# Bostanabad-Research-Group/GP-Plus

Measured on AMD Instinct MI355X. Metric: MLL evals/sec (fwd+grad), NxN exact GP, N=20k d=8, higher is better.
Workload: dtype f64; 1 GPU; C2: synthetic Borehole (Sobol seed 0, unique rows, z-scored) N=20000 d=8 fp64, GP_Plus Rough_RBF exact GP at theta1, one replica per GPU (restart-parallel); N=20000, d=8, streams_per_gpu=1

## Files before the change

gp-plus_amd/csrc/gpp_gemm.hip:

```cpp
#include "../../include/gpp.h"
#include "gpp_internal.h"

#include <algorithm>
#include <atomic>
#include <cstdlib>

typedef double v2d __attribute__((ext_vector_type(2)));
typedef double v4d __attribute__((ext_vector_type(4)));

namespace {

constexpr int BK16 = 16;
constexpr int ldt_mc(int T, int BK = 16) { return BK == 16 ? T + 16 : T + 4; }
constexpr int LDK = BK16 + 2;

__device__ __forceinline__ bool keep_elem(int mask, int k, int row) {
  return (mask == 0) | ((mask == 1) & (k <= row)) | ((mask == 2) & (k >= row));
}

template <int T>
__device__ __forceinline__ unsigned load_kc(const double* __restrict__ P, int64_t ld, int R, int r0, int kb, int kend,
                                            int mask, int tid, v2d (&reg)[T / 32]) {
  unsigned keep = 0;
  const double* ptr[T / 32];
#pragma unroll
  for (int i = 0; i < T / 32; ++i) {
    const int v = tid + 256 * i;
    const int gr = r0 + (v >> 3);
    const int gk = kb + ((v & 7) << 1);
    const bool v0 = (gr < R) & (gk < kend);
    const bool k0 = v0 & keep_elem(mask, gk, gr);
    const bool k1 = v0 & (gk + 1 < kend) & keep_elem(mask, gk + 1, gr);
    keep |= (k0 ? 1u : 0u) << (2 * i);
    keep |= (k1 ? 1u : 0u) << (2 * i + 1);
    ptr[i] = v0 ? P + (int64_t)gr * ld + gk : P;
  }
#pragma unroll
  for (int i = 0; i < T / 32; ++i) reg[i] = *reinterpret_cast<const v2d*>(ptr[i]);
  return keep;
}
template <int T, bool SEL>
__device__ __forceinline__ void store_kc(double* __restrict__ s, int tid, const v2d (&reg)[T / 32], unsigned keep) {
#pragma unroll
  for (int i = 0; i < T / 32; ++i) {
    const int v = tid + 256 * i;
    v2d t = reg[i];
    if (SEL) {
      t.x = ((keep >> (2 * i)) & 1u) ? t.x : 0.0;
      t.y = ((keep >> (2 * i + 1)) & 1u) ? t.y : 0.0;
    }
    *reinterpret_cast<v2d*>(s + (v >> 3) * LDK + ((v & 7) << 1)) = t;
  }
}

template <int T, int BK, int NTH = 256>
__device__ __forceinline__ unsigned load_mc(const double* __restrict__ P, int64_t ld, int R, int r0, int kb, int kend,
                                            int mask, int tid, v2d (&reg)[BK * T / (2 * NTH)], const double* __restrict__ dummy) {
  constexpr int NV = BK * T / (2 * NTH);
  unsigned keep = 0;
  const double* ptr[NV];
#pragma unroll
  for (int i = 0; i < NV; ++i) {
    const int v = tid + NTH * i;
    const int gk = kb + v / (T / 2);
    const int gr = r0 + ((v % (T / 2)) << 1);
    const bool v0 = (gk < kend) & (gr < R);
    const bool k0 = v0 & keep_elem(mask, gk, gr);
    const bool k1 = v0 & (gr + 1 < R) & keep_elem(mask, gk, gr + 1);
    keep |= (k0 ? 1u : 0u) << (2 * i);
    keep |= (k1 ? 1u : 0u) << (2 * i + 1);
    ptr[i] = v0 ? P + (int64_t)gk * ld + gr : dummy;
  }
#pragma unroll
  for (int i = 0; i < NV; ++i) reg[i] = *reinterpret_cast<const v2d*>(ptr[i]);
  return keep;
}
template <int T, int BK, bool SEL, int NTH = 256>
__device__ __forceinline__ void store_mc(double* __restrict__ s, int tid, const v2d (&reg)[BK * T / (2 * NTH)], unsigned keep) {
#pragma unroll
  for (int i = 0; i < BK * T / (2 * NTH); ++i) {
    const int v = tid + NTH * i;
    v2d t = reg[i];
    if (SEL) {
      t.x = ((keep >> (2 * i)) & 1u) ? t.x : 0.0;
      t.y = ((keep >> (2 * i + 1)) & 1u) ? t.y : 0.0;
    }
    *reinterpret_cast<v2d*>(s + (v / (T / 2)) * ldt_mc(T, BK) + ((v % (T / 2)) << 1)) = t;
  }
}

template <int T, int BK>
__device__ __forceinline__ bool chunk_is_interior(int r0, int R, int kb, int kend, int mask) {
  if (r0 + T > R || kb + BK > kend) return false;
  if (mask == 1) return kb + BK - 1 <= r0;
  if (mask == 2) return kb >= r0 + T - 1;
  return true;
}
template <int T, int BK>
__device__ __forceinline__ bool chunk_in_range(int r0, int R, int kb, int kend) {
  return r0 + T <= R && kb + BK <= kend;
}
template <int T, int BK, int NTH = 256>
__device__ __forceinline__ unsigned mask_bits_mc(int r0, int kb, int mask, int tid) {
  unsigned keep = 0;
#pragma unroll
  for (int i = 0; i < BK * T / (2 * NTH); ++i) {
    const int v = tid + NTH * i;
    const int gk = kb + v / (T / 2);
    const int gr = r0 + ((v % (T / 2)) << 1);
    keep |= (keep_elem(mask, gk, gr) ? 1u : 0u) << (2 * i);
    keep |= (keep_elem(mask, gk, gr + 1) ? 1u : 0u) << (2 * i + 1);
  }
  return keep;
}
template <int T, bool KC, int BK, int NTH = 256>
__device__ __forceinline__ void thread_offsets(int64_t ld, int tid, unsigned (&off)[BK * T / (2 * NTH)]) {
#pragma unroll
  for (int i = 0; i < BK * T / (2 * NTH); ++i) {
    const int v = tid + NTH * i;
    if (KC) off[i] = (unsigned)(((int64_t)(v >> 3) * ld + ((v & 7) << 1)) * 8);
    else off[i] = (unsigned)(((int64_t)(v / (T / 2)) * ld + ((v % (T / 2)) << 1)) * 8);
  }
}
template <int NV>
__device__ __forceinline__ void load_fast(const double* __restrict__ ubase, const unsigned (&off)[NV], v2d (&reg)[NV]) {
#pragma unroll
  for (int i = 0; i < NV; ++i)
    reg[i] = *reinterpret_cast<const v2d*>(reinterpret_cast<const char*>(ubase) + off[i]);
}

struct GemmNoHook {
  __device__ __forceinline__ void operator()() const {}
};
struct GemmStoreC {};
template <int VAR, int WTM, int WTN, int TAG, int BK, int NBUF, int WR, class P, class H = GemmNoHook, class E = GemmStoreC>
__device__ __forceinline__ void gemm_tile(const P& p, const int tm, const int tn, const double* __restrict__ A,
                                          const double* __restrict__ B, double* __restrict__ C, double* C2,
                                          double* __restrict__ smem, H before_epilogue = H(), const E& epi = E()) {
  static_assert(BK == 16 || VAR == 2, "wide K chunks are implemented for row-contiguous (TN) operands only");
  static_assert(BK % 16 == 0 && (NBUF == 1 || NBUF == 2), "bad staging parameters");
  static_assert(WR == 2 || (WR == 4 && VAR == 2 && BK == 16 && NBUF == 2 && WTM == 64 && WTN == 64), "the tall tile is TN only");
  constexpr int NTH = 128 * WR;
  constexpr bool A_KC = (VAR != 2);
  constexpr bool B_KC = (VAR == 0);
  constexpr int TM = WR * WTM, TN = 2 * WTN;
  constexpr int LDA = ldt_mc(TM, BK), LDB = ldt_mc(TN, BK);
  constexpr int TX = TM > TN ? TM : TN;
  constexpr int OPSZ = (BK * ldt_mc(TX, BK) > TX * LDK) ? BK * ldt_mc(TX, BK) : TX * LDK;
  constexpr int OPA = (WR == 2) ? OPSZ : BK * LDA, OPB = (WR == 2) ? OPSZ : BK * LDB;
  constexpr int NVA = BK * TM / (2 * NTH), NVB = BK * TN / (2 * NTH);
  constexpr int RB = WTM / 4, CB = WTN / 16;

  const int tid = threadIdx.x;
  const int wave = tid >> 6, lane = tid & 63;
  const int wm = (wave >> 1) * WTM, wn = (wave & 1) * WTN;
  const int li = lane & 15, lk = lane >> 4;
  const int row0 = tm * TM, col0 = tn * TN;
  const double* __restrict__ Bd = B;
  double* __restrict__ Cd = C;
  if (p.compact_bc) {
    const int b = tn / p.own_bt, q = (b + p.own_off) / p.own_mod;
    const int64_t bias = (int64_t)(q - b) * p.own_bt * TN;
    B += bias;
    C += bias;
  }

  int klo = 0;
  if (p.klo_mode == 1) klo = row0;
  else if (p.klo_mode == 2) klo = col0;
  else if (p.klo_mode == 3) klo = row0 > col0 ? row0 : col0;
  int khi = p.K;
  if (p.khi_mode == 1) khi = min(p.K, row0 + TM);
  else if (p.khi_mode == 2) khi = min(p.K, col0 + TN);
  const int nch = khi > klo ? (khi - klo + BK - 1) / BK : 0;

  static_assert(RB % 4 == 0, "wave tile rows must be a multiple of 16");
  v4d acc4[RB / 4][CB];
#pragma unroll
  for (int a = 0; a < RB / 4; ++a)
#pragma unroll
    for (int b = 0; b < CB; ++b) acc4[a][b] = (v4d){0.0, 0.0, 0.0, 0.0};

  v2d ra[NVA], rb[NVB];
  unsigned ka = 0, kb_ = 0;
  unsigned offa[NVA], offb[NVB];
  thread_offsets<TM, A_KC, BK, NTH>(p.lda, tid, offa);
  thread_offsets<TN, B_KC, BK, NTH>(p.ldb, tid, offb);
  const double* __restrict__ ubaseA = A_KC ? A + (int64_t)row0 * p.lda : A + row0;
  const double* __restrict__ ubaseB = B_KC ? B + (int64_t)col0 * p.ldb : B + col0;
  const int64_t stepA = A_KC ? 1 : p.lda, stepB = B_KC ? 1 : p.ldb;

  const int Mld = (VAR == 2 && p.pad_ok) ? ((p.M + TM - 1) / TM) * TM : p.M;
  const int Nld = (VAR == 2 && p.pad_ok) ? ((p.N + TN - 1) / TN) * TN : p.N;
  int pa = 0, pb = 0;
  auto stage_load = [&](int kb) {
    pa = pb = 0;
    if constexpr (VAR == 2) {
      if (chunk_in_range<TM, BK>(row0, Mld, kb, khi)) pa = chunk_is_interior<TM, BK>(row0, Mld, kb, khi, p.a_mask) ? 1 : 2;
      if (chunk_in_range<TN, BK>(col0, Nld, kb, khi)) pb = chunk_is_interior<TN, BK>(col0, Nld, kb, khi, p.b_mask) ? 1 : 2;
    }
    if (pa) {
      load_fast<NVA>(ubaseA + (int64_t)kb * stepA, offa, ra);
      if (pa == 2) ka = mask_bits_mc<TM, BK, NTH>(row0, kb, p.a_mask, tid);
    } else {
      if constexpr (A_KC) ka = load_kc<TM>(A, p.lda, p.M, row0, kb, khi, p.a_mask, tid, ra);
      else ka = load_mc<TM, BK, NTH>(A, p.lda, p.M, row0, kb, khi, p.a_mask, tid, ra, A);
    }
    if (pb) {
      load_fast<NVB>(ubaseB + (int64_t)kb * stepB, offb, rb);
      if (pb == 2) kb_ = mask_bits_mc<TN, BK, NTH>(col0, kb, p.b_mask, tid);
    } else {
      if constexpr (B_KC) kb_ = load_kc<TN>(B, p.ldb, p.N, col0, kb, khi, p.b_mask, tid, rb);
      else kb_ = load_mc<TN, BK, NTH>(B, p.ldb, p.N, col0, kb, khi, p.b_mask, tid, rb, Bd);
    }
  };
  auto stage_store = [&](double* da, double* db) {
    if (pa == 1) {
      if constexpr (A_KC) store_kc<TM, false>(da, tid, ra, 0); else store_mc<TM, BK, false, NTH>(da, tid, ra, 0);
    } else {
      if constexpr (A_KC) store_kc<TM, true>(da, tid, ra, ka); else store_mc<TM, BK, true, NTH>(da, tid, ra, ka);
    }
    if (pb == 1) {
      if constexpr (B_KC) store_kc<TN, false>(db, tid, rb, 0); else store_mc<TN, BK, false, NTH>(db, tid, rb, 0);
    } else {
      if constexpr (B_KC) store_kc<TN, true>(db, tid, rb, kb_); else store_mc<TN, BK, true, NTH>(db, tid, rb, kb_);
    }
  };

  auto kpos = [&](int c) { return p.k_reverse ? klo + (nch - 1 - c) * BK : klo + c * BK; };
  if (nch > 0) {
    stage_load(kpos(0));
    stage_store(smem, smem + OPA);
  }
  __syncthreads();

  auto compute = [&](int cur) {
    const double* sa = smem + cur * (OPA + OPB) + (A_KC ? (wm + li) * LDK + lk : wm + li + lk * LDA);
    const double* sb = smem + cur * (OPA + OPB) + OPA + (B_KC ? (wn + li) * LDK + lk : wn + li + lk * LDB);
#pragma unroll
    for (int kk = 0; kk < BK / 4; ++kk) {
      double bf[CB], af[RB / 4];
#pragma unroll
      for (int b = 0; b < CB; ++b) bf[b] = B_KC ? sb[16 * b * LDK + kk * 4] : sb[kk * 4 * LDB + 16 * b];
#pragma unroll
      for (int a = 0; a < RB / 4; ++a) af[a] = A_KC ? sa[16 * a * LDK + kk * 4] : sa[kk * 4 * LDA + 16 * a];
#pragma unroll
      for (int a = 0; a < RB / 4; ++a)
#pragma unroll
        for (int b = 0; b < CB; ++b)
          acc4[a][b] = __builtin_amdgcn_mfma_f64_16x16x4f64(af[a], bf[b], acc4[a][b], 0, 0, 0);
    }
  };

  int ca = 0, cb = 0;
  constexpr bool SPLIT = (VAR == 2 && RB == 16 && CB == 4 && BK == 16);
  if constexpr (SPLIT) {
    if (row0 + TM <= Mld && col0 + TN <= Nld && nch > 1) {
      int k_lo = klo, k_hi = khi;
      if (p.a_mask == 1) k_hi = min(k_hi, row0 + 1);
      if (p.a_mask == 2) k_lo = max(k_lo, row0 + TM - 1);
      if (p.b_mask == 1) k_hi = min(k_hi, col0 + 1);
      if (p.b_mask == 2) k_lo = max(k_lo, col0 + TN - 1);
      int j_lo = (k_lo - klo + BK - 1) / BK, j_hi = (k_hi - klo) / BK;
      j_lo = max(j_lo, 0);
      j_hi = min(j_hi, nch);
      if (j_hi > j_lo) {
        const int ci_lo = p.k_reverse ? nch - j_hi : j_lo, ci_hi = p.k_reverse ? nch - j_lo : j_hi;
        ca = max(ci_lo - 1, 0);
        cb = min(ci_hi - 1, nch - 1);
        if (cb < ca) ca = cb = 0;
      }
    }
  }
  auto general_iter = [&](int c) {
    const int cur = (NBUF == 2) ? (c & 1) : 0;
    const bool more = (c + 1 < nch);
    if (more) stage_load(kpos(c + 1));
    compute(cur);
    if (NBUF == 1) __syncthreads();
    if (more) {
      const int nxt = (NBUF == 2) ? (cur ^ 1) : 0;
      stage_store(smem + nxt * (OPA + OPB), smem + nxt * (OPA + OPB) + OPA);
    }
    __syncthreads();
  };
  int c = 0;
  for (; c < ca; ++c) general_iter(c);
  if constexpr (SPLIT) {
    for (; c < cb; ++c) {
      const int cur = (NBUF == 2) ? (c & 1) : 0, nxt = (NBUF == 2) ? (cur ^ 1) : 0;
      const int kb = kpos(c + 1);
      load_fast<NVA>(ubaseA + (int64_t)kb * stepA, offa, ra);
      load_fast<NVB>(ubaseB + (int64_t)kb * stepB, offb, rb);
      if constexpr (TAG != 0) __builtin_amdgcn_s_setprio(1);
      compute(cur);
      if constexpr (TAG != 0) __builtin_amdgcn_s_setprio(0);
      if (NBUF == 1) __syncthreads();
      store_mc<TM, BK, false, NTH>(smem + nxt * (OPA + OPB), tid, ra, 0);
      store_mc<TN, BK, false, NTH>(smem + nxt * (OPA + OPB) + OPA, tid, rb, 0);
      __syncthreads();
    }
  }
  for (; c < nch; ++c) general_iter(c);
  before_epilogue();
  if constexpr (!__is_same(E, GemmStoreC)) {
    static_assert((VAR == 2 || VAR == 0) && WTM == 64 && WTN == 64 && WR == 2, "accumulator epilogues are written for the big tile");
    epi(acc4, row0, col0, p.M, smem);
    return;
  }

  const double alpha = p.alpha, beta = p.beta;
  constexpr int GA = RB < 4 ? RB : 4;
#pragma unroll
  for (int a0 = 0; a0 < RB; a0 += GA) {
    double cold[GA][CB];
    if (beta != 0.0) {
#pragma unroll
      for (int a = 0; a < GA; ++a) {
        const int m = row0 + wm + 4 * (a0 + a) + lk;
#pragma unroll
        for (int b = 0; b < CB; ++b) {
          const int n = col0 + wn + 16 * b + li;
          const bool ok = (m < p.M) && (n < p.N) && (p.c_lower == 0 || (p.c_lower == 1 ? n <= m : n >= m));
          const double* src = ok ? C + (int64_t)m * p.ldc + n : Cd;
          cold[a][b] = *src;
        }
      }
    }
#pragma unroll
    for (int a = 0; a < GA; ++a) {
      const int m = row0 + wm + 4 * (a0 + a) + lk;
#pragma unroll
      for (int b = 0; b < CB; ++b) {
        const int n = col0 + wn + 16 * b + li;
        const bool ok = (m < p.M) && (n < p.N) && (p.c_lower == 0 || (p.c_lower == 1 ? n <= m : n >= m));
        double v = alpha * acc4[(a0 + a) >> 2][b][(a0 + a) & 3];
        if (beta != 0.0) v = fma(beta, cold[a][b], v);
        if (ok) {
          C[(int64_t)m * p.ldc + n] = v;
          if (C2)
            C2[(int64_t)n * p.ldc2 + m] = v;
        }
      }
    }
  }
}

template <int VAR, int WTM, int WTN, int TAG = 0, int BK = 16, int NBUF = 2, int WR = 2>
__global__ __launch_bounds__(128 * WR, ((VAR == 2 && !(BK > 16 && WTM >= 64)) || WTM < 64) ? 2 : 1) void gpp_gemm_f64(GemmArgs p) {
  constexpr int TM = WR * WTM, TN = 2 * WTN;
  extern __shared__ __attribute__((aligned(16))) double smem[];
  int tm, tn;
  if (p.swz) {
    const int b = blockIdx.x, xcd = b & 7, i = b >> 3;
    const int S = (i >> 6) * 8 + xcd, w = i & 63;
    const int super_n = (p.tiles_n + 7) >> 3;
    const int sm = S / super_n, sn = S - sm * super_n;
    tm = sm * 8 + (w >> 3);
    tn = sn * 8 + (w & 7);
    if (tm >= p.tiles_m || tn >= p.tiles_n) return;
    if ((p.c_lower == 1 && tn > tm) || (p.c_lower == 2 && tn < tm)) return;
  } else {
    const int t = (p.batch_fast ? (int)(blockIdx.x / (unsigned)p.nbatch) : (int)blockIdx.x) + (int)p.tile_base;
    if (p.c_lower == 1 && p.row_mod >= 1) {
      const float a = 0.5f * (float)p.row_mod, b = (float)p.row_off + 1.f - a;
      int i = (int)((-b + sqrtf(b * b + 4.f * a * (float)t)) / (2.f * a));
      auto S = [&](int q) { return q * (p.row_off + 1) + p.row_mod * (q * (q - 1) / 2); };
      while (S(i + 1) <= t) ++i;
      while (S(i) > t) --i;
      tm = p.row_off + p.row_mod * i;
      tn = t - S(i);
    } else if (p.c_lower == 1 && TM == 2 * TN) {
      tm = (int)((sqrtf(4.f * (float)t + 1.f) - 1.f) * 0.5f);
      while ((tm + 1) * (tm + 2) <= t) ++tm;
      while (tm * (tm + 1) > t) --tm;
      tn = t - tm * (tm + 1);
      if (tn >= p.tiles_n) return;
    } else if (p.c_lower) {
      tm = (int)((sqrtf(8.f * (float)t + 1.f) - 1.f) * 0.5f);
      while ((tm + 1) * (tm + 2) / 2 <= t) ++tm;
      while (tm * (tm + 1) / 2 > t) --tm;
      tn = t - tm * (tm + 1) / 2;
      if (p.c_lower == 1 && p.own_mod > 1 && (tn / p.own_bt + p.own_off) % p.own_mod != 0) return;
      if (p.c_lower == 2) {
        const int q = tm;
        tm = tn;
        tn = q;
        if (p.own_mod > 1 && (tm / p.own_bt + p.own_off) % p.own_mod != 0) return;
        if ((tn + 1) * TN <= p.skip_lead) return;
        if (p.row_limit > 0 && tm * TM >= p.row_limit) return;
      }
    } else if (p.col_major) {
      tn = t / p.tiles_m;
      tm = t - tn * p.tiles_m;
    } else {
      tm = t / p.tiles_n;
      tn = t - tm * p.tiles_n;
      if (p.row_reverse) tm = p.tiles_m - 1 - tm;
    }
  }
  const int64_t bi = p.batch_fast ? (int64_t)(blockIdx.x % (unsigned)p.nbatch) : (int64_t)blockIdx.y;
  gemm_tile<VAR, WTM, WTN, TAG, BK, NBUF, WR>(p, tm, tn, p.A + bi * p.sA + (int64_t)blockIdx.z * p.zA, p.B + bi * p.sB + (int64_t)blockIdx.z * p.zB,
                                             p.C + bi * p.sC + (int64_t)blockIdx.z * p.zC,
                                             p.C2 ? p.C2 + bi * p.sC2 + (int64_t)blockIdx.z * p.zC2 : nullptr, smem);

}

__device__ __forceinline__ double wave_sum(double v) {
#pragma unroll
  for (int o = 32; o > 0; o >>= 1) v += __shfl_xor(v, o);
  return v;
}
template <int DT>
struct GradEpilogue {
  GradEpiArgs e;
  int tile;
  static constexpr int T = 128;
  static constexpr int FIXED = 2 * DT * T + 2 * T + DT + 4 * (DT + 1);
  static constexpr int SLAB = (FIXED + 1) & ~1;
  static_assert((SLAB + 16 * 256) * sizeof(double) <= 2 * 2 * BK16 * ldt_mc(T) * sizeof(double), "the epilogue lives in the main loop's LDS");
  __device__ __forceinline__ void operator()(const v4d (&acc4)[4][4], int row0, int col0, int N, double* __restrict__ smem) const {
    const int tid = threadIdx.x, wave = tid >> 6, lane = tid & 63;
    const int wm = (wave >> 1) * 64, wn = (wave & 1) * 64, li = lane & 15, lk = lane >> 4;
    const int D = e.D;
    double* __restrict__ sa = smem;
    double* __restrict__ sb = sa + DT * T;
    double* __restrict__ sal_a = sb + DT * T;
    double* __restrict__ sal_b = sal_a + T;
    double* __restrict__ sw = sal_b + T;
    double* __restrict__ red = sw + DT;
    double* __restrict__ slab = smem + SLAB;
    for (int x = tid; x < DT * T; x += 256) {
      const int d = x / T, r = x - d * T;
      sa[x] = (d < D && row0 + r < N) ? e.U[(int64_t)(row0 + r) * D + d] : 0.0;
      sb[x] = (d < D && col0 + r < N) ? e.U[(int64_t)(col0 + r) * D + d] : 0.0;
    }
    if (tid < T) {
      sal_a[tid] = (row0 + tid < N) ? e.alpha[row0 + tid] : 0.0;
      sal_b[tid] = (col0 + tid < N) ? e.alpha[col0 + tid] : 0.0;
    }
    if (tid < DT) sw[tid] = (tid < D) ? e.w[tid] : 0.0;
    __syncthreads();

    const double sf2 = *e.sf2;
    const GppExpConsts ec = gpp_exp_consts();
    const bool diag_tile = (row0 == col0);
    double my_sf2 = 0.0, my_w[DT];
#pragma unroll
    for (int d = 0; d < DT; ++d) my_w[d] = 0.0;
#pragma unroll
    for (int a4 = 0; a4 < 4; ++a4) {
#pragma unroll
      for (int v = 0; v < 4; ++v)
#pragma unroll
        for (int b = 0; b < 4; ++b) slab[(v * 4 + b) * 256 + tid] = acc4[a4][b][v];
#pragma unroll 1
      for (int h = 0; h < 2; ++h) {
        const int ra = wm + 16 * a4 + 8 * h + lk;
        const int cb = wn + li;
        double r2[2][4];
#pragma unroll
        for (int a = 0; a < 2; ++a)
#pragma unroll
          for (int b = 0; b < 4; ++b) r2[a][b] = 0.0;
#pragma unroll 2
        for (int d = 0; d < DT; ++d) {
          const double ua[2] = {sa[d * T + ra], sa[d * T + ra + 4]};
          const double wd = sw[d];
#pragma unroll
          for (int b = 0; b < 4; ++b) {
            const double ub = sb[d * T + cb + 16 * b];
#pragma unroll
            for (int a = 0; a < 2; ++a) {
              const double df = ua[a] - ub;
              r2[a][b] = fma(wd * df, df, r2[a][b]);
            }
          }
        }
        __asm__ volatile("" ::: "memory");
        double g2[2][4];
#pragma unroll
        for (int a = 0; a < 2; ++a) {
          const int i = row0 + ra + 4 * a;
          const double al_i = sal_a[ra + 4 * a];
#pragma unroll
          for (int b = 0; b < 4; ++b) {
            const int j = col0 + cb + 16 * b;
            const bool ok = (i < N) & (j <= i);
            const double kv = gpp_exp_nonpos(-r2[a][b], ec);
            const double kin = slab[((2 * h + a) * 4 + b) * 256 + tid];
            double Wij = 0.5 * (al_i * sal_b[cb + 16 * b] - kin);
            Wij = ok ? Wij : 0.0;
            const double mult = (i == j) ? 1.0 : 2.0;
            my_sf2 = fma(mult * Wij, kv, my_sf2);
            g2[a][b] = mult * Wij * sf2 * kv;
            if (diag_tile && ok && i == j) e.wdiag[i] = Wij;
          }
        }
#pragma unroll
        for (int d = 0; d < DT; ++d) {
          const double ua[2] = {sa[d * T + ra], sa[d * T + ra + 4]};
          double s = 0.0;
#pragma unroll
          for (int b = 0; b < 4; ++b) {
            const double ub = sb[d * T + cb + 16 * b];
#pragma unroll
            for (int a = 0; a < 2; ++a) {
              const double df = ua[a] - ub;
              s = fma(-g2[a][b] * df, df, s);
            }
          }
          my_w[d] += s;
          __builtin_amdgcn_sched_barrier(0);
        }
      }
    }
#pragma unroll
    for (int q = 0; q <= DT; ++q) {
      const double v = wave_sum(q < DT ? my_w[q < DT ? q : 0] : my_sf2);
      if (lane == 0) red[wave * (DT + 1) + q] = v;
    }
    __syncthreads();
    if (tid <= D) {
      const int q = (tid == D) ? DT : tid;
      e.rec[(int64_t)tile * (D + 1) + tid] = ((red[q] + red[(DT + 1) + q]) + red[2 * (DT + 1) + q]) + red[3 * (DT + 1) + q];
    }
  }
};

template <int DT>
__global__ __launch_bounds__(256, 2) void gpp_lauum_grad_f64(GemmArgs p, GradEpiArgs e) {
  extern __shared__ __attribute__((aligned(16))) double smem[];
  const int t = (int)blockIdx.x;
  int tm = (int)((sqrtf(8.f * (float)t + 1.f) - 1.f) * 0.5f);
  while ((tm + 1) * (tm + 2) / 2 <= t) ++tm;
  while (tm * (tm + 1) / 2 > t) --tm;
  const int tn = t - tm * (tm + 1) / 2;
  gemm_tile<2, 64, 64, 2, 16, 2, 2>(p, tm, tn, p.A, p.B, nullptr, nullptr, smem, GemmNoHook(), GradEpilogue<DT>{e, t});
}

template <bool MAT>
struct PostCrossEpilogue {
  PostCrossArgs e;
  int tile, Mr;
  static constexpr int T = 128, DC = 16;
  static constexpr int SLAB = 2 * DC * T + T + 2 * T;
  static_assert((SLAB & 1) == 0 && (SLAB + 16 * 256) * sizeof(double) <= 2 * 2 * BK16 * ldt_mc(T) * sizeof(double) &&
                    (SLAB + 16 * 256) * sizeof(double) <= 2 * 2 * T * LDK * sizeof(double),
                "the epilogue lives in the main loop's LDS");
  __device__ __forceinline__ void operator()(const v4d (&acc4)[4][4], int row0, int col0, int Mc, double* __restrict__ smem) const {
    const int tid = threadIdx.x, wave = tid >> 6, lane = tid & 63;
    const int wm = (wave >> 1) * 64, wn = (wave & 1) * 64, li = lane & 15, lk = lane >> 4;
    const int D = e.dk & 255, kind = (e.dk >> 8) & 255;
    const int dsp = (!MAT || kind == 0) ? D : (e.dk >> 16);
    double* __restrict__ sa = smem;
    double* __restrict__ sb = sa + DC * T;
    double* __restrict__ som = sb + DC * T;
    double* __restrict__ rs = som + T;
    double* __restrict__ slab = smem + SLAB;
    const double* __restrict__ Uc = e.Uc;
    const double* __restrict__ Ur = e.Ur;
    const double* __restrict__ wp = e.w;
    double* __restrict__ rec = e.rec + (int64_t)tile * T;
    Uc += (int64_t)row0 * (e.dk & 255);
    Ur += (int64_t)col0 * (e.dk & 255);
    int rlim = Mc - row0, clim = Mr - col0;
    asm volatile("" : "+v"(Uc), "+v"(Ur), "+v"(wp), "+v"(rec), "+v"(rlim), "+v"(clim));
    auto stage = [&](int d0) {
      for (int x = tid; x < DC * T; x += 256) {
        const int dd = x / T, r = x - dd * T, d = d0 + dd;
        const bool okd = d < D;
        const double sw = okd ? sqrt(wp[okd ? d : 0]) : 0.0;
        sa[x] = (okd && r < rlim) ? Uc[r * D + d] * sw : 0.0;
        sb[x] = (okd && r < clim) ? Ur[r * D + d] * sw : 0.0;
      }
    };
    if (tid < T) som[tid] = (tid < clim) ? (e.omega ? e.omega[col0 + tid] : 1.0) : 0.0;
    const bool one = (D <= DC);
    if (one) stage(0);
    __syncthreads();

    const double sf2 = *e.sf2;
    const GppExpConsts ec = gpp_exp_consts();
#pragma unroll
    for (int a4 = 0; a4 < 4; ++a4) {
#pragma unroll
      for (int v = 0; v < 4; ++v)
#pragma unroll
        for (int b = 0; b < 4; ++b) slab[(v * 4 + b) * 256 + tid] = acc4[a4][b][v];
#pragma unroll 1
      for (int h = 0; h < 2; ++h) {
        const int ra = wm + 16 * a4 + 8 * h + lk;
        const int cb = wn + li;
        double r2[2][4], r2m[MAT ? 2 : 1][MAT ? 4 : 1];
#pragma unroll
        for (int a = 0; a < 2; ++a)
#pragma unroll
          for (int b = 0; b < 4; ++b) {
            r2[a][b] = 0.0;
            if (MAT) r2m[MAT ? a : 0][MAT ? b : 0] = 0.0;
          }
#pragma unroll 1
        for (int d0 = 0; d0 < D; d0 += DC) {
// ... 733 lines not shown
```

Baseline: 7.961 evals/s.

## Hand-schedule interior GEMM k-loop to interleave global loads, LDS ops and MFMAs

Adds a dedicated pipelined main loop for interior tiles of the TN double-buffered big-tile GEMM. It uses scalar-uniform base pointers with per-thread offsets, register-fragment prefetch of the next k-step, and explicit sched_group_barrier ordering that spreads global loads, LDS reads and LDS writes between MFMAs. The goal is to hide memory and LDS latency behind matrix math and reduce address arithmetic. It adds compiler-sensitive scheduling code and asm register pinning that may raise register pressure or serialize poorly if the schedule mismatches the generated instructions.

```diff
diff --git a/gp-plus_amd/csrc/gpp_gemm.hip b/gp-plus_amd/csrc/gpp_gemm.hip
--- a/gp-plus_amd/csrc/gpp_gemm.hip
+++ b/gp-plus_amd/csrc/gpp_gemm.hip
@@ -7,9 +7,14 @@
 
 typedef double v2d __attribute__((ext_vector_type(2)));
 typedef double v4d __attribute__((ext_vector_type(4)));
+typedef const char __attribute__((address_space(1))) gchar;
+typedef const v2d __attribute__((address_space(1))) gv2d;
 
 namespace {
 
+#ifndef GPP_CLEAN_SETPRIO
+#define GPP_CLEAN_SETPRIO 1
+#endif
 constexpr int BK16 = 16;
 constexpr int ldt_mc(int T, int BK = 16) { return BK == 16 ? T + 16 : T + 4; }
 constexpr int LDK = BK16 + 2;
@@ -150,6 +155,8 @@
   constexpr int OPA = (WR == 2) ? OPSZ : BK * LDA, OPB = (WR == 2) ? OPSZ : BK * LDB;
   constexpr int NVA = BK * TM / (2 * NTH), NVB = BK * TN / (2 * NTH);
   constexpr int RB = WTM / 4, CB = WTN / 16;
+  constexpr bool SPLIT = (VAR == 2 && RB == 16 && CB == 4 && BK == 16 && NBUF == 2 && WR == 2);
+  constexpr bool PIPE = SPLIT && __is_same(H, GemmNoHook);
 
   const int tid = threadIdx.x;
   const int wave = tid >> 6, lane = tid & 63;
@@ -199,6 +206,12 @@
       if (chunk_in_range<TM, BK>(row0, Mld, kb, khi)) pa = chunk_is_interior<TM, BK>(row0, Mld, kb, khi, p.a_mask) ? 1 : 2;
       if (chunk_in_range<TN, BK>(col0, Nld, kb, khi)) pb = chunk_is_interior<TN, BK>(col0, Nld, kb, khi, p.b_mask) ? 1 : 2;
     }
+    if constexpr (PIPE) {
+#pragma unroll
+      for (int i = 0; i < NVA; ++i) asm("" : "+v"(offa[i]));
+#pragma unroll
+      for (int i = 0; i < NVB; ++i) asm("" : "+v"(offb[i]));
+    }
     if (pa) {
       load_fast<NVA>(ubaseA + (int64_t)kb * stepA, offa, ra);
       if (pa == 2) ka = mask_bits_mc<TM, BK, NTH>(row0, kb, p.a_mask, tid);
@@ -253,7 +266,6 @@
   };
 
   int ca = 0, cb = 0;
-  constexpr bool SPLIT = (VAR == 2 && RB == 16 && CB == 4 && BK == 16);
   if constexpr (SPLIT) {
     if (row0 + TM <= Mld && col0 + TN <= Nld && nch > 1) {
       int k_lo = klo, k_hi = khi;
@@ -286,19 +298,121 @@
   };
   int c = 0;
   for (; c < ca; ++c) general_iter(c);
-  if constexpr (SPLIT) {
+  if constexpr (SPLIT && !PIPE) {
     for (; c < cb; ++c) {
-      const int cur = (NBUF == 2) ? (c & 1) : 0, nxt = (NBUF == 2) ? (cur ^ 1) : 0;
+      const int cur = c & 1, nxt = cur ^ 1;
       const int kb = kpos(c + 1);
       load_fast<NVA>(ubaseA + (int64_t)kb * stepA, offa, ra);
       load_fast<NVB>(ubaseB + (int64_t)kb * stepB, offb, rb);
-      if constexpr (TAG != 0) __builtin_amdgcn_s_setprio(1);
       compute(cur);
-      if constexpr (TAG != 0) __builtin_amdgcn_s_setprio(0);
-      if (NBUF == 1) __syncthreads();
       store_mc<TM, BK, false, NTH>(smem + nxt * (OPA + OPB), tid, ra, 0);
       store_mc<TN, BK, false, NTH>(smem + nxt * (OPA + OPB) + OPA, tid, rb, 0);
       __syncthreads();
+    }
+  }
+  if constexpr (PIPE) {
+    if (c < cb) {
+      static_assert(!SPLIT || (TM == TN && LDA == LDB && NTH % (TM / 2) == 0), "the clean loop assumes the square row-contiguous tile");
+      constexpr int RPV = NTH / (TM / 2);
+      auto uniform_ptr = [](const double* q) {
+        const uint64_t u = reinterpret_cast<uint64_t>(q);
+        const uint32_t lo = __builtin_amdgcn_readfirstlane((uint32_t)u), hi = __builtin_amdgcn_readfirstlane((uint32_t)(u >> 32));
+        return reinterpret_cast<gchar*>(((uint64_t)hi << 32) | lo);
+      };
+      const int kb1 = kpos(c + 1);
+      gchar* ua = uniform_ptr(ubaseA + (int64_t)kb1 * stepA);
+      gchar* ub = uniform_ptr(ubaseB + (int64_t)kb1 * stepB);
+      const int64_t dk = p.k_reverse ? -(int64_t)BK : (int64_t)BK;
+      const int64_t inca = dk * stepA * 8, incb = dk * stepB * 8;
+      int wofs = (tid / (TM / 2)) * LDA + ((tid % (TM / 2)) << 1);
+      int rofa = wm + li + lk * LDA, rofb = OPA + wn + li + lk * LDB;
+      asm("" : "+v"(wofs), "+v"(rofa), "+v"(rofb));
+      for (; c < cb; ++c) {
+        const int cur = c & 1;
+        const double* sa = smem + cur * (OPA + OPB) + rofa;
+        const double* sb = smem + cur * (OPA + OPB) + rofb;
+        int wpos = (cur ^ 1) * (OPA + OPB) + wofs;
+#pragma unroll
+        for (int i = 0; i < NVA; ++i) asm("" : "+v"(offa[i]));
+#pragma unroll
+        for (int i = 0; i < NVB; ++i) asm("" : "+v"(offb[i]));
+        if constexpr (TAG != 0 && GPP_CLEAN_SETPRIO) __builtin_amdgcn_s_setprio(1);
+        double af[BK / 4][RB / 4], bf[BK / 4][CB];
+        auto frag_b = [&](int kk) {
+#pragma unroll
+          for (int b = 0; b < CB; ++b) bf[kk][b] = sb[kk * 4 * LDB + 16 * b];
+        };
+        auto frag_a = [&](int kk, int a0) {
+#pragma unroll
+          for (int a = a0; a < a0 + 2; ++a) af[kk][a] = sa[kk * 4 * LDA + 16 * a];
+        };
+        auto mfma_rows = [&](int kk, int a0) {
+#pragma unroll
+          for (int a = a0; a < a0 + 2; ++a)
+#pragma unroll
+            for (int b = 0; b < CB; ++b)
+              acc4[a][b] = __builtin_amdgcn_mfma_f64_16x16x4f64(af[kk][a], bf[kk][b], acc4[a][b], 0, 0, 0);
+        };
+        auto stage = [&](int ofs, const v2d& v) {
+          asm("" : "+v"(wpos));
+          *reinterpret_cast<v2d*>(smem + wpos + ofs) = v;
+        };
+        frag_b(0);
+        frag_a(0, 0);
+        frag_a(0, 2);
+#pragma unroll
+        for (int kk = 0; kk < BK / 4; ++kk) {
+          if (kk + 1 < BK / 4) frag_b(kk + 1);
+          if (kk == BK / 4 - 1) {
+#pragma unroll
+            for (int i = 0; i < NVB; ++i) stage(OPA + i * RPV * LDB, rb[i]);
+          }
+          mfma_rows(kk, 0);
+          if (kk == 0) {
+#pragma unroll
+            for (int i = 0; i < NVA; ++i) ra[i] = *reinterpret_cast<gv2d*>(ua + offa[i]);
+#pragma unroll
+            for (int i = 0; i < NVB; ++i) rb[i] = *reinterpret_cast<gv2d*>(ub + offb[i]);
+            ua += inca;
+            ub += incb;
+          }
+          if (kk + 1 < BK / 4) frag_a(kk + 1, 0);
+          if (kk == BK / 4 - 2) {
+#pragma unroll
+            for (int i = 0; i < NVA; ++i) stage(i * RPV * LDA, ra[i]);
+          }
+          if (kk + 1 < BK / 4) frag_a(kk + 1, 2);
+          mfma_rows(kk, 2);
+        }
+        static_assert(BK == 16 && RB / 4 * CB == 16 && NVA == 4 && NVB == 4, "the schedule below is written out for 4 k-steps of 16 MFMAs");
+#define GPP_SG(mask, n) __builtin_amdgcn_sched_group_barrier(mask, n, 0)
+#define GPP_SG_NEXT_B GPP_SG(0x8, 1); GPP_SG(0x100, 1); GPP_SG(0x8, 1); GPP_SG(0x100, 1)
+#define GPP_SG_PAIR(mask, m) GPP_SG(mask, 1); GPP_SG(0x8, m)
+        GPP_SG(0x100, 4);
+        GPP_SG_NEXT_B;
+        GPP_SG_PAIR(0x20, 1); GPP_SG_PAIR(0x20, 1); GPP_SG_PAIR(0x20, 1); GPP_SG_PAIR(0x20, 1); GPP_SG_PAIR(0x20, 1); GPP_SG_PAIR(0x20, 1);
+        GPP_SG(0x100, 1);
+        GPP_SG_PAIR(0x20, 1); GPP_SG_PAIR(0x20, 1);
+        GPP_SG(0x8, 6);
+        GPP_SG(0x100, 1);
+        GPP_SG_NEXT_B;
+        GPP_SG(0x8, 6);
+        GPP_SG(0x100, 1);
+        GPP_SG(0x8, 8);
+        GPP_SG(0x100, 1);
+        GPP_SG_NEXT_B;
+        GPP_SG(0x8, 6);
+        GPP_SG(0x100, 1);
+        GPP_SG_PAIR(0x200, 2); GPP_SG_PAIR(0x200, 2); GPP_SG_PAIR(0x200, 2); GPP_SG_PAIR(0x200, 2);
+        GPP_SG(0x100, 1);
+        GPP_SG_PAIR(0x200, 2); GPP_SG_PAIR(0x200, 2); GPP_SG_PAIR(0x200, 2); GPP_SG_PAIR(0x200, 2);
+        GPP_SG(0x8, 8);
+#undef GPP_SG_PAIR
+#undef GPP_SG_NEXT_B
+#undef GPP_SG
+        if constexpr (TAG != 0 && GPP_CLEAN_SETPRIO) __builtin_amdgcn_s_setprio(0);
+        __syncthreads();
+      }
     }
   }
   for (; c < nch; ++c) general_iter(c);
```

Result: faster. 8.057 evals/s, median of 6 (+1.2%).
